# buwantaiji/DominantSparseEigenAD

Hardware: AMD Instinct MI355X
Metric: DominantSparseSymeig fwd+bwd ms & HBM GB/s (TFIM, fp64) (higher is better)
Workload: dtype f64

## Files before the change

dominantsparseeigenad_amd/csrc/dsea_kernels.hip:

```cpp
#include <hip/hip_runtime.h>
#include <hip/hip_ext.h>
#include <stdint.h>

#include <type_traits>

#include "dsea_internal.h"
#include "dsea_device.h"

namespace dsea {

__global__ __launch_bounds__(256) void k_finalize1(const double* __restrict__ partials, int count,
                                                   double* __restrict__ out) {
  __shared__ double sm4[4];
  double acc = 0.0;
  for (int b = threadIdx.x; b < count; b += 256) acc += partials[b];
  double t = block_sum(acc, sm4);
  if (threadIdx.x == 0) out[0] = t;
}

__global__ __launch_bounds__(256) void k_finalize_pair(const double* __restrict__ PA, int na, double* __restrict__ outA,
                                                       const double* __restrict__ PB, int nb, double* __restrict__ outB,
                                                       const double* __restrict__ skipB) {
  __shared__ double sm4[4];
  const bool second = blockIdx.x == 1;
  if (second && skipB && skipB[0] != 0.0) return;
  const double* __restrict__ P = second ? PB : PA;
  const int count = second ? nb : na;
  double acc = 0.0;
  for (int b = threadIdx.x; b < count; b += 256) acc += P[b];
  double t = block_sum(acc, sm4);
  if (threadIdx.x == 0) (second ? outB : outA)[0] = t;
}

template <bool GATE>
__global__ __launch_bounds__(256) void k_finalize_multi(const double* __restrict__ P, int64_t pstride,
                                                        int nw, double* __restrict__ c,
                                                        const double* __restrict__ brk,
                                                        const double* __restrict__ gate) {
  __shared__ double sm4[4];
  const double gate0 = GATE ? gate[0] : 1.0;
  if (broken(brk)) return;
  if (GATE && gate0 == 0.0) return;
  const int j = blockIdx.x;
  const double* __restrict__ row = P + (int64_t)j * pstride;
  double a0 = 0.0, a1 = 0.0, a2 = 0.0, a3 = 0.0;
  int w = threadIdx.x;
  for (; w + 768 < nw; w += 1024) {
    a0 += row[w];
    a1 += row[w + 256];
    a2 += row[w + 512];
    a3 += row[w + 768];
  }
  for (; w < nw; w += 256) a0 += row[w];
  double t = block_sum((a0 + a1) + (a2 + a3), sm4);
  if (threadIdx.x == 0) c[j] = t;
}

template <int NP>
struct RdotsPre {
  double2 uu[NP], qa[NP], qb[NP];
};

template <int RPL, bool GUARD, bool PRE, bool USCALE = false>
__device__ __forceinline__ void rdots_tile(const double* __restrict__ Q, int64_t ldq, int i, int ii, int64_t n,
                                           int64_t base, int lane, const double* __restrict__ u,
                                           double a, double b, double* __restrict__ r,
                                           double* __restrict__ sP, bool accumulate, bool want_rr,
                                           const RdotsPre<RPL / 2>& pre, double usc = 1.0) {
  constexpr int NP = RPL / 2;
  double2 rv[NP];
  const double* __restrict__ q1 = Q + (int64_t)(i - 1) * ldq;
  const double* __restrict__ q2 = (i >= 2) ? Q + (int64_t)(i - 2) * ldq : nullptr;
#pragma unroll
  for (int t = 0; t < NP; ++t) {
    const int64_t row = base + t * 128 + lane * 2;
    double2 uu, qa, qb;
    if (PRE) {
      uu = pre.uu[t];
      qa = pre.qa[t];
      qb = pre.qb[t];
    } else {
      uu = ld2<GUARD>(u, row, n);
      qa = ld2<GUARD>(q1, row, n);
      qb = make_double2(0.0, 0.0);
      if (q2) qb = ld2<GUARD>(q2, row, n);
    }
    if (USCALE) {
      uu.x = uu.x / usc;
      uu.y = uu.y / usc;
    }
    rv[t].x = __dsub_rn(__dsub_rn(uu.x, __dmul_rn(a, qa.x)), __dmul_rn(b, qb.x));
    rv[t].y = __dsub_rn(__dsub_rn(uu.y, __dmul_rn(a, qa.y)), __dmul_rn(b, qb.y));
  }
  if (want_rr) {
    double acc = 0.0;
#pragma unroll
    for (int t = 0; t < NP; ++t) {
      acc = fma(rv[t].x, rv[t].x, acc);
      acc = fma(rv[t].y, rv[t].y, acc);
    }
    acc = wave_sum(acc);
    if (lane == 0) sP[i] = accumulate ? (sP[i] + acc) : acc;
  }
  const int nchunks = ii / 4;
  const bool rev = (i & 1) != 0;
  auto single = [&](int j) {
    const double* __restrict__ qj = Q + (int64_t)j * ldq;
    double acc = 0.0;
#pragma unroll
    for (int t = 0; t < NP; ++t) {
      double2 q = ld2_stream<GUARD>(qj, base + t * 128 + lane * 2, n);
      acc = fma(q.x, rv[t].x, acc);
      acc = fma(q.y, rv[t].y, acc);
    }
    acc = wave_sum(acc);
    if (lane == 0) sP[j] = accumulate ? (sP[j] + acc) : acc;
  };
  if (rev)
    for (int j = ii - 1; j >= 4 * nchunks; --j) single(j);
  for (int cc = 0; cc < nchunks; ++cc) {
    const int j = 4 * (rev ? nchunks - 1 - cc : cc);
    const double* __restrict__ qj = Q + (int64_t)j * ldq;
    double2 q[4][NP];
#pragma unroll
    for (int v = 0; v < 4; ++v)
#pragma unroll
      for (int t = 0; t < NP; ++t) q[v][t] = ld2_stream<GUARD>(qj + (int64_t)v * ldq, base + t * 128 + lane * 2, n);
    double acc[4];
#pragma unroll
    for (int v = 0; v < 4; ++v) {
      acc[v] = 0.0;
#pragma unroll
      for (int t = 0; t < NP; ++t) {
        acc[v] = fma(q[v][t].x, rv[t].x, acc[v]);
        acc[v] = fma(q[v][t].y, rv[t].y, acc[v]);
      }
    }
    const double bsum = wave_sum4_rows(acc[0], acc[1], acc[2], acc[3]);
    if ((lane & 15) == 15) {
      const int idx = j + (lane >> 4);
      sP[idx] = accumulate ? (sP[idx] + bsum) : bsum;
    }
  }
  if (!rev)
    for (int j = 4 * nchunks; j < ii; ++j) single(j);
#pragma unroll
  for (int t = 0; t < NP; ++t) st2<GUARD>(r, base + t * 128 + lane * 2, n, rv[t]);
}

template <int RPL, bool SEL = false, bool USCALE = false>
__global__ __launch_bounds__(256) void k_rdots(const double* __restrict__ Q, int64_t ldq, int i,
                                               int64_t n, const double* __restrict__ u,
                                               const double* __restrict__ alpha,
                                               const double* __restrict__ beta, double* __restrict__ r,
                                               double* __restrict__ P, int64_t pstride, int nw,
                                               int64_t ntiles, const double* __restrict__ aP, int aCount,
                                               double* __restrict__ a_store, int want_rr,
                                               double* __restrict__ brk, const double* __restrict__ sel,
                                               int sel_exit, const double* __restrict__ uscale) {
  const int lane = threadIdx.x & 63;
  const int wpb = blockDim.x >> 6;
  if (SEL && sel_exit && sel[0] == 0.0) return;
  const int64_t widx = (int64_t)blockIdx.x * wpb + (threadIdx.x >> 6);
  constexpr int64_t TILE = 64 * RPL;
  extern __shared__ double rdots_lds[];
  double* __restrict__ sP = rdots_lds + (threadIdx.x >> 6) * (i + 1);
  const int cnt = i + (want_rr ? 1 : 0);
  RdotsPre<RPL / 2> pre;
  const bool pre_ok = widx < nw && widx * TILE + TILE <= n;
  if (pre_ok) {
    const double* __restrict__ q1 = Q + (int64_t)(i - 1) * ldq;
    const double* __restrict__ q2 = (i >= 2) ? Q + (int64_t)(i - 2) * ldq : nullptr;
#pragma unroll
    for (int t = 0; t < RPL / 2; ++t) {
      const int64_t row = widx * TILE + t * 128 + lane * 2;
      pre.uu[t] = ld2<false>(u, row, n);
      pre.qa[t] = ld2<false>(q1, row, n);
      pre.qb[t] = make_double2(0.0, 0.0);
      if (q2) pre.qb[t] = ld2<false>(q2, row, n);
    }
  }
  if (broken(brk)) return;
  if (widx < nw) {
    double a;
    if (aCount > 0) {
      a = sum_partials_wave(aP, aCount, lane);
      if (widx == 0 && lane == 0) a_store[0] = a;
    } else {
      a = alpha[0];
    }
    const double b = beta ? beta[0] : 0.0;
    const double usc = USCALE ? uscale[0] : 1.0;
    if (brk && widx == 0 && lane == 0) brk[1] = fmax(brk[1], fmax(fabs(a), fabs(b)));
    const int ii = (SEL && sel[0] == 0.0) ? 0 : i;
    bool first = true;
    for (int64_t tile = widx; tile < ntiles; tile += nw) {
      const int64_t base = tile * TILE;
      if (first && pre_ok)
        rdots_tile<RPL, false, true, USCALE>(Q, ldq, i, ii, n, base, lane, u, a, b, r, sP, false, want_rr != 0, pre, usc);
      else if (base + TILE <= n)
        rdots_tile<RPL, false, false, USCALE>(Q, ldq, i, ii, n, base, lane, u, a, b, r, sP, !first, want_rr != 0, pre, usc);
      else
        rdots_tile<RPL, true, false, USCALE>(Q, ldq, i, ii, n, base, lane, u, a, b, r, sP, !first, want_rr != 0, pre, usc);
      first = false;
    }
  } else {
    for (int idx = lane; idx < cnt; idx += 64) sP[idx] = 0.0;
  }
  __syncthreads();
  const int row0 = (SEL && sel[0] == 0.0) ? i : 0;
  for (int idx = row0 + threadIdx.x; idx < cnt; idx += blockDim.x) {
    double t = rdots_lds[idx];
    for (int w = 1; w < wpb; ++w) t += rdots_lds[w * (i + 1) + idx];
    P[(int64_t)idx * pstride + blockIdx.x] = t;
  }
}

template <int RPL, bool GUARD, int MODE>
__device__ __forceinline__ double axpy_tile(const double* __restrict__ Q, int64_t ldq, int i, int64_t n,
                                            int64_t base, int lane, const double* __restrict__ c,
                                            double* __restrict__ r) {
  constexpr int NP = RPL / 2;
  double2 w[NP];
#pragma unroll
  for (int t = 0; t < NP; ++t) w[t] = make_double2(0.0, 0.0);
#pragma unroll 4
  for (int jj = 0; jj < i; ++jj) {
    const int j = i - 1 - jj;
    const double* __restrict__ qj = Q + (int64_t)j * ldq;
    const double cj = c[j];
#pragma unroll
    for (int t = 0; t < NP; ++t) {
      const int64_t row = base + t * 128 + lane * 2;
      double2 q = ld2_stream<GUARD>(qj, row, n);
      w[t].x = fma(cj, q.x, w[t].x);
      w[t].y = fma(cj, q.y, w[t].y);
    }
  }
  double acc = 0.0;
#pragma unroll
  for (int t = 0; t < NP; ++t) {
    const int64_t row = base + t * 128 + lane * 2;
    if (MODE == 0) {
      double2 rv = ld2<GUARD>(r, row, n);
      rv.x -= w[t].x;
      rv.y -= w[t].y;
      st2<GUARD>(r, row, n, rv);
      acc = fma(rv.x, rv.x, acc);
      acc = fma(rv.y, rv.y, acc);
    } else {
      st2<GUARD>(r, row, n, w[t]);
    }
  }
  return acc;
}

template <int RPL, int MODE, bool SEL = false>
__global__ __launch_bounds__(256) void k_axpy_norm(const double* __restrict__ Q, int64_t ldq, int i,
                                                   int64_t n, const double* __restrict__ c,
                                                   double* __restrict__ r, double* __restrict__ P,
                                                   int nw, int64_t ntiles, const double* __restrict__ brk,
                                                   const double* __restrict__ sel) {
  const int lane = threadIdx.x & 63;
  const int64_t widx = (int64_t)blockIdx.x * 4 + (threadIdx.x >> 6);
  if (widx >= nw) return;
  const double sel0 = SEL ? sel[0] : 1.0;
  if (broken(brk)) return;
  if (SEL && sel0 == 0.0) {
    if (MODE == 0 && lane == 0) P[widx] = (widx == 0) ? c[i] : 0.0;
    return;
  }
  constexpr int64_t TILE = 64 * RPL;
  double acc = 0.0;
  for (int64_t tile = widx; tile < ntiles; tile += nw) {
    const int64_t base = tile * TILE;
    if (base + TILE <= n)
      acc += axpy_tile<RPL, false, MODE>(Q, ldq, i, n, base, lane, c, r);
    else
      acc += axpy_tile<RPL, true, MODE>(Q, ldq, i, n, base, lane, c, r);
  }
  if (MODE == 0) {
    acc = wave_sum(acc);
    if (lane == 0) P[widx] = acc;
  }
}

template <int W, int NT, bool SEL = false>
__global__ __launch_bounds__(W * 64) void k_rdots_split(const double* __restrict__ Q, int64_t ldq, int i,
                                                        int64_t n, const double* __restrict__ u,
                                                        const double* __restrict__ alpha,
                                                        const double* __restrict__ beta, double* __restrict__ r,
                                                        double* __restrict__ P, int64_t pstride,
                                                        const double* __restrict__ aP, int aCount,
                                                        double* __restrict__ a_store, int want_rr,
                                                        double* __restrict__ brk, const double* __restrict__ sel,
                                                        int sel_exit) {
  if (SEL && sel_exit && sel[0] == 0.0) return;
  const int lane = threadIdx.x & 63, wv = threadIdx.x >> 6;
// ... 776 lines not shown
    if (row != row0) v = ld2<true>(r, row, n);
    v.x = v.x / beta;
    v.y = v.y / beta;
    st2<true>(fa.q_out, row, n, v);
    if (fa.qs_out) st_bf16x2(fa.qs_out, row, n, v);
  }
}

__device__ __forceinline__ double tfim_diag(const TfimParams& p, int64_t i, uint64_t maskL) {
  const uint64_t gi = (uint64_t)(p.row_offset + i);
  const uint64_t rot = ((gi << 1) | (gi >> (p.L - 1))) & maskL;
  const int pop = __popcll(gi ^ rot);
  return p.diag_scale * (double)(-(p.L - 2 * pop));
}

template <int T, bool FUSED>
__global__ __launch_bounds__(256) void k_spmv_tfim(TfimParams p, const double* __restrict__ x,
                                                   double* __restrict__ y,
                                                   const double* __restrict__ shift,
                                                   const double* __restrict__ skip,
                                                   double* __restrict__ P, TfimFusedArgs fa) {
  constexpr int TILE = 1 << T;
  constexpr int NPAIR = TILE / 2;
  constexpr int PER = (NPAIR + 255) / 256;
#ifndef DSEA_FB_FUSED
#define DSEA_FB_FUSED 7
#endif
#ifndef DSEA_FB_PLAIN
#define DSEA_FB_PLAIN 9
#endif
  constexpr int FB = PER >= 4 ? (FUSED ? DSEA_FB_FUSED : DSEA_FB_PLAIN) : (PER == 2 ? 12 : 14);
  __shared__ double2 tile2[NPAIR];
  __shared__ double sm5[5];
  if (!FUSED && skip && skip[0] != 0.0) return;
  if (FUSED && broken(fa.brk)) return;
  const uint64_t maskL = (p.L >= 64) ? ~0ull : ((1ull << p.L) - 1ull);
  const int64_t ntiles = ((int64_t)1 << p.L_local) >> T;
  double acc = 0.0;
  double beta = 1.0, g = 0.0, s = 0.0;
  bool first = true;
  for (int64_t tile = blockIdx.x; tile < ntiles; tile += gridDim.x) {
    const int64_t base = tile * TILE;
    double2 own[PER];
    double2 fb[PER][FB];
#pragma unroll
    for (int t = 0; t < PER; ++t) {
      const int lp = t * 256 + threadIdx.x;
      const int64_t i0 = base + 2 * (int64_t)(lp < NPAIR ? lp : 0);
      own[t] = *reinterpret_cast<const double2*>(x + i0);
#pragma unroll
      for (int e = 0; e < FB; ++e) {
        fb[t][e] = make_double2(0.0, 0.0);
        if (T + e < p.L_local) fb[t][e] = *reinterpret_cast<const double2*>(x + (i0 ^ ((int64_t)1 << (T + e))));
      }
    }
    if (first) {
      if (FUSED && !fused_beta(fa, sm5, beta)) return;
      g = p.g_dev ? p.g_dev[0] : p.g_const;
      s = shift ? shift[0] : 0.0;
      first = false;
    }
    __syncthreads();
#pragma unroll
    for (int t = 0; t < PER; ++t) {
      const int lp = t * 256 + threadIdx.x;
      if (lp < NPAIR) {
        double2 v = own[t];
        if (FUSED) {
          v.x = v.x / beta;
          v.y = v.y / beta;
          *reinterpret_cast<double2*>(fa.q_out + base + 2 * lp) = v;
          if (fa.qs_out)
            *reinterpret_cast<uint32_t*>(fa.qs_out + base + 2 * lp) =
                (uint32_t)f64_to_bf16(v.x) | ((uint32_t)f64_to_bf16(v.y) << 16);
        }
        tile2[lp] = v;
      }
    }
    __syncthreads();
    double2 far[PER];
#pragma unroll
    for (int t = 0; t < PER; ++t) {
      far[t] = make_double2(0.0, 0.0);
#pragma unroll
      for (int e = 0; e < FB; ++e) {
        far[t].x += fb[t][e].x;
        far[t].y += fb[t][e].y;
      }
    }
    int j = T + FB;
    for (; j + 4 <= p.L_local; j += 4) {
      double2 nb[PER][4];
#pragma unroll
      for (int t = 0; t < PER; ++t) {
        const int lp = t * 256 + threadIdx.x;
        const int64_t i0 = base + 2 * (int64_t)(lp < NPAIR ? lp : 0);
#pragma unroll
        for (int e = 0; e < 4; ++e)
          nb[t][e] = *reinterpret_cast<const double2*>(x + (i0 ^ ((int64_t)1 << (j + e))));
      }
#pragma unroll
      for (int t = 0; t < PER; ++t) {
        far[t].x += (nb[t][0].x + nb[t][1].x) + (nb[t][2].x + nb[t][3].x);
        far[t].y += (nb[t][0].y + nb[t][1].y) + (nb[t][2].y + nb[t][3].y);
      }
    }
    for (; j < p.L_local; ++j) {
#pragma unroll
      for (int t = 0; t < PER; ++t) {
        const int lp = t * 256 + threadIdx.x;
        const int64_t i0 = base + 2 * (int64_t)(lp < NPAIR ? lp : 0);
        const double2 nbv = *reinterpret_cast<const double2*>(x + (i0 ^ ((int64_t)1 << j)));
        far[t].x += nbv.x;
        far[t].y += nbv.y;
      }
    }
#pragma unroll
    for (int t = 0; t < PER; ++t) {
      const int lp = t * 256 + threadIdx.x;
      if (lp < NPAIR) {
        const int64_t i0 = base + 2 * (int64_t)lp;
        const double2 xv = tile2[lp];
        double2 sum = make_double2(xv.y, xv.x);
#pragma unroll
        for (int jb = 1; jb < T; ++jb) {
          const double2 nbv = tile2[lp ^ (1 << (jb - 1))];
          sum.x += nbv.x;
          sum.y += nbv.y;
        }
        if (FUSED) {
          sum.x += far[t].x / beta;
          sum.y += far[t].y / beta;
        } else {
          sum.x += far[t].x;
          sum.y += far[t].y;
        }
        double2 v;
        v.x = __dsub_rn(__dmul_rn(xv.x, tfim_diag(p, i0, maskL)), __dmul_rn(g, sum.x));
        v.y = __dsub_rn(__dmul_rn(xv.y, tfim_diag(p, i0 + 1, maskL)), __dmul_rn(g, sum.y));
        if (!FUSED && shift) {
          v.x = __dsub_rn(v.x, __dmul_rn(s, xv.x));
          v.y = __dsub_rn(v.y, __dmul_rn(s, xv.y));
        }
        *reinterpret_cast<double2*>(y + i0) = v;
        acc = fma(xv.x, v.x, acc);
        acc = fma(xv.y, v.y, acc);
      }
    }
  }
  if (P) {
    __syncthreads();
    double tot = block_sum(acc, sm5);
    if (threadIdx.x == 0) P[blockIdx.x] = tot;
  }
}

__global__ void k_spmv_tfim_single(TfimParams p, const double* __restrict__ x, double* __restrict__ y,
                                   const double* __restrict__ shift, const double* __restrict__ skip,
                                   double* __restrict__ P) {
  if (skip && skip[0] != 0.0) return;
  const uint64_t maskL = (p.L >= 64) ? ~0ull : ((1ull << p.L) - 1ull);
  const double xi = x[0];
  double v = __dmul_rn(xi, tfim_diag(p, 0, maskL));
  if (shift) v = __dsub_rn(v, __dmul_rn(shift[0], xi));
  y[0] = v;
  if (P) P[0] = xi * v;
}

__global__ __launch_bounds__(256) void k_cg_update_fused(double* __restrict__ x, double* __restrict__ r,
                                                         const double* __restrict__ d,
                                                         const double* __restrict__ Ad,
                                                         const double* __restrict__ state, int parity,
                                                         const double* __restrict__ dP, int dCount,
                                                         int64_t n, double* __restrict__ P) {
  __shared__ double sm5[5];
  const int64_t stride = (int64_t)gridDim.x * 512;
  const int64_t row0 = ((int64_t)blockIdx.x * 256 + threadIdx.x) * 2;
  double2 xv = ld2<true>(x, row0, n), rv = ld2<true>(r, row0, n);
  double2 dv = ld2<true>(d, row0, n), av = ld2<true>(Ad, row0, n);
  if (state[DSEA_CG_DONE] != 0.0) return;
  const double dAd = sum_partials_block(dP, dCount, sm5);
  const double alpha = state[parity ? DSEA_CG_RRNEW : DSEA_CG_RR] / dAd;
  double acc = 0.0;
  for (int64_t row = row0; row < n; row += stride) {
    if (row != row0) {
      xv = ld2<true>(x, row, n);
      rv = ld2<true>(r, row, n);
      dv = ld2<true>(d, row, n);
      av = ld2<true>(Ad, row, n);
    }
    xv.x = __dadd_rn(xv.x, __dmul_rn(alpha, dv.x));
    xv.y = __dadd_rn(xv.y, __dmul_rn(alpha, dv.y));
    rv.x = __dsub_rn(rv.x, __dmul_rn(alpha, av.x));
    rv.y = __dsub_rn(rv.y, __dmul_rn(alpha, av.y));
    st2<true>(x, row, n, xv);
    st2<true>(r, row, n, rv);
    acc = fma(rv.x, rv.x, acc);
    acc = fma(rv.y, rv.y, acc);
  }
  __syncthreads();
  double t = block_sum(acc, sm5);
  if (threadIdx.x == 0) P[blockIdx.x] = t;
}

__global__ __launch_bounds__(256) void k_cg_direction_fused(const double* __restrict__ r,
                                                            double* __restrict__ d,
                                                            double* __restrict__ state, int parity,
                                                            const double* __restrict__ rP, int rCount,
                                                            double eps, int64_t n) {
  __shared__ double sm5[5];
  const int64_t stride = (int64_t)gridDim.x * 512;
  const int64_t row0 = ((int64_t)blockIdx.x * 256 + threadIdx.x) * 2;
  double2 rv = ld2<true>(r, row0, n), dv = ld2<true>(d, row0, n);
  if (state[DSEA_CG_DONE] != 0.0) return;
  const double rr_new = sum_partials_block(rP, rCount, sm5);
  const double rr = state[parity ? DSEA_CG_RRNEW : DSEA_CG_RR];
  const double rn = sqrt(rr_new);
  const bool conv = rn < eps;
  if (blockIdx.x == 0 && threadIdx.x == 0) {
    state[DSEA_CG_ITERS] += 1.0;
    state[DSEA_CG_RESNORM] = rn;
    if (conv) state[DSEA_CG_DONE] = 1.0;
    else state[parity ? DSEA_CG_RR : DSEA_CG_RRNEW] = rr_new;
  }
  if (conv) return;
  const double beta = rr_new / rr;
  for (int64_t row = row0; row < n; row += stride) {
    if (row != row0) {
      rv = ld2<true>(r, row, n);
      dv = ld2<true>(d, row, n);
    }
    dv.x = __dadd_rn(rv.x, __dmul_rn(beta, dv.x));
    dv.y = __dadd_rn(rv.y, __dmul_rn(beta, dv.y));
    st2<true>(d, row, n, dv);
  }
}

template <int G>
__global__ __launch_bounds__(256) void k_spmv_csr(CsrParams p, const double* __restrict__ x,
                                                  double* __restrict__ y,
                                                  const double* __restrict__ shift,
                                                  const double* __restrict__ skip,
                                                  double* __restrict__ P) {
  __shared__ double sm4[4];
  if (skip && skip[0] != 0.0) return;
  const double s = shift ? shift[0] : 0.0;
  const int sub = threadIdx.x % G;
  const int64_t rows_per_block = 256 / G;
  double acc = 0.0;
  for (int64_t row = (int64_t)blockIdx.x * rows_per_block + threadIdx.x / G; row < p.n;
       row += (int64_t)gridDim.x * rows_per_block) {
    const int64_t lo = p.rowptr[row], hi = p.rowptr[row + 1];
    double sum = 0.0;
    for (int64_t e = lo + sub; e < hi; e += G) sum = fma(p.vals[e], x[p.colidx[e]], sum);
#pragma unroll
    for (int m = G / 2; m >= 1; m >>= 1) sum += __shfl_xor(sum, m, 64);
    if (sub == 0) {
      const double xi = x[row];
      double v = sum;
      if (shift) v = __dsub_rn(v, __dmul_rn(s, xi));
      y[row] = v;
      acc = fma(xi, v, acc);
    }
  }
  if (P) {
    double tot = block_sum(acc, sm4);
    if (threadIdx.x == 0) P[blockIdx.x] = tot;
  }
}

#define CSR_ROWS 128
#define CSR_CAP 6144
__global__ __launch_bounds__(256) void k_spmv_csr_stream(CsrParams p, const double* __restrict__ x,
                                                         double* __restrict__ y,
                                                         const double* __restrict__ shift,
                                                         const double* __restrict__ skip,
                                                         double* __restrict__ P) {
  __shared__ double prod[CSR_CAP];
  __shared__ double sm4[4];
  if (skip && skip[0] != 0.0) return;
  const double s = shift ? shift[0] : 0.0;
  double acc = 0.0;
  const int64_t nchunks = (p.n + CSR_ROWS - 1) / CSR_ROWS;
  for (int64_t chunk = blockIdx.x; chunk < nchunks; chunk += gridDim.x) {
    const int64_t r0 = chunk * CSR_ROWS;
    const int64_t r1 = (r0 + CSR_ROWS < p.n) ? r0 + CSR_ROWS : p.n;
    const int64_t e0 = p.rowptr[r0], e1 = p.rowptr[r1];
    __syncthreads();
    if (e1 - e0 <= CSR_CAP) {
      for (int64_t e = e0 + threadIdx.x; e < e1; e += 256) prod[e - e0] = p.vals[e] * x[p.colidx[e]];
      __syncthreads();
      const int64_t row = r0 + threadIdx.x;
      if (threadIdx.x < CSR_ROWS && row < r1) {
        const int lo = (int)(p.rowptr[row] - e0), hi = (int)(p.rowptr[row + 1] - e0);
        double sum = 0.0;
        for (int e = lo; e < hi; ++e) sum += prod[e];
        const double xi = x[row];
        double v = sum;
        if (shift) v = __dsub_rn(v, __dmul_rn(s, xi));
        y[row] = v;
        acc = fma(xi, v, acc);
      }
    } else {
      const int sub = threadIdx.x & 31;
      for (int64_t row = r0 + (threadIdx.x >> 5); row < r1; row += 8) {
        double sum = 0.0;
// ... 1354 lines not shown
  const double* nullc = nullptr;
  if (g.split_w) {
    const unsigned tiles = (unsigned)g.ntiles;
    EventPair* ev = nullptr;
    switch (g.split_w) {
      case 4: KLAUNCH(ev, (k_axpy_norm_split<4, 1>), tiles, 256, st, Q, ldq, k, n, s, out, nullP, nullc, nullc); break;
      case 8: KLAUNCH(ev, (k_axpy_norm_split<8, 1>), tiles, 512, st, Q, ldq, k, n, s, out, nullP, nullc, nullc); break;
      default: KLAUNCH(ev, (k_axpy_norm_split<16, 1>), tiles, 1024, st, Q, ldq, k, n, s, out, nullP, nullc, nullc); break;
    }
    return;
  }
  const int grid = (g.nw + 3) / 4;
  switch (g.rpl) {
    case 2: hipLaunchKernelGGL((k_axpy_norm<2, 1>), dim3(grid), dim3(256), 0, st, Q, ldq, k, n, s, out, nullP, g.nw, g.ntiles, nullc, nullc); break;
    case 4: hipLaunchKernelGGL((k_axpy_norm<4, 1>), dim3(grid), dim3(256), 0, st, Q, ldq, k, n, s, out, nullP, g.nw, g.ntiles, nullc, nullc); break;
    case 8: hipLaunchKernelGGL((k_axpy_norm<8, 1>), dim3(grid), dim3(256), 0, st, Q, ldq, k, n, s, out, nullP, g.nw, g.ntiles, nullc, nullc); break;
    default: hipLaunchKernelGGL((k_axpy_norm<16, 1>), dim3(grid), dim3(256), 0, st, Q, ldq, k, n, s, out, nullP, g.nw, g.ntiles, nullc, nullc); break;
  }
}

__global__ __launch_bounds__(256) void k_probe_read(const double* __restrict__ x, int64_t n, double* __restrict__ P) {
  __shared__ double sm4[4];
  double acc = 0.0;
  for (int64_t base = (int64_t)blockIdx.x * 4096; base < n; base += (int64_t)gridDim.x * 4096) {
    double2 v[8];
#pragma unroll
    for (int t = 0; t < 8; ++t) v[t] = ld2_stream<true>(x, base + t * 512 + threadIdx.x * 2, n);
#pragma unroll
    for (int t = 0; t < 8; ++t) acc += v[t].x + v[t].y;
  }
  const double tot = block_sum(acc, sm4);
  if (threadIdx.x == 0) P[blockIdx.x] = tot;
}

__global__ __launch_bounds__(256) void k_probe_copy(const double* __restrict__ x, double* __restrict__ y, int64_t n) {
  for (int64_t base = (int64_t)blockIdx.x * 4096; base < n; base += (int64_t)gridDim.x * 4096) {
    double2 v[8];
#pragma unroll
    for (int t = 0; t < 8; ++t) v[t] = ld2_stream<true>(x, base + t * 512 + threadIdx.x * 2, n);
#pragma unroll
    for (int t = 0; t < 8; ++t) st2<true>(y, base + t * 512 + threadIdx.x * 2, n, v[t]);
  }
}

void launch_probe(const double* x, double* y, int64_t n, double* P, int nP, hipStream_t st) {
  int64_t tiles = (n + 4095) / 4096;
  const int grid = (int)(tiles < nP ? tiles : nP);
  if (y)
    hipLaunchKernelGGL(k_probe_copy, dim3(grid), dim3(256), 0, st, x, y, n);
  else
    hipLaunchKernelGGL(k_probe_read, dim3(grid), dim3(256), 0, st, x, n, P);
}

void launch_dot(const double* x, const double* y, int64_t n, double* P, double* out, hipStream_t st) {
  const int nb = ew_blocks(n);
  hipLaunchKernelGGL(k_dot, dim3(nb), dim3(256), 0, st, x, y, n, P);
  launch_finalize1(P, nb, out, st);
}

void launch_shift_dot(const double* x, double* y, const double* shift, const double* skip, int64_t n,
                      double* P, double* out, hipStream_t st) {
  const int nb = ew_blocks(n);
  hipLaunchKernelGGL(k_shift_dot, dim3(nb), dim3(256), 0, st, x, y, shift, skip, n, P);
  hipLaunchKernelGGL(k_cg_finalize_slot, dim3(1), dim3(256), 0, st, (const double*)P, nb, out, skip);
}

int launch_shift_dot_partials(const double* x, double* y, const double* shift, const double* skip, int64_t n, double* P,
                              hipStream_t st) {
  const int nb = ew_blocks(n);
  hipLaunchKernelGGL(k_shift_dot, dim3(nb), dim3(256), 0, st, x, y, shift, skip, n, P);
  return nb;
}

void launch_axpy(double a_host, const double* a_dev, const double* x, double* y, int64_t n,
                 hipStream_t st) {
  hipLaunchKernelGGL(k_axpy, dim3(ew_blocks(n)), dim3(256), 0, st, a_host, a_dev, x, y, n);
}

void launch_scale_store_fused(const double* r, const double* nP, int nCount, double* q, uint16_t* qs, double* beta_store,
                              int64_t n, hipStream_t st) {
  TfimFusedArgs fa = {nP, nCount, q, qs, beta_store, nullptr, 0};
  hipLaunchKernelGGL(k_scale_store_fused, dim3(ew_blocks(n)), dim3(256), 0, st, r, fa, n);
}

int launch_dot_partials(const double* x, const double* y, int64_t n, double* P, hipStream_t st) {
  const int nb = ew_blocks(n);
  hipLaunchKernelGGL(k_dot, dim3(nb), dim3(256), 0, st, x, y, n, P);
  return nb;
}

void launch_scale_store(const double* r, const double* nrm2, double* q, double* beta_out, int64_t n,
                        hipStream_t st, uint16_t* qs, double* brk, int step) {
  hipLaunchKernelGGL(k_scale_store, dim3(ew_blocks(n)), dim3(256), 0, st, r, nrm2, q, beta_out, n, qs, brk, step);
}

void launch_project_apply(const double* v, const double* a, const double* dot, double* out, int64_t n,
                          hipStream_t st) {
  hipLaunchKernelGGL(k_project_apply, dim3(ew_blocks(n)), dim3(256), 0, st, v, a, dot, out, n);
}

void launch_cg_init(const double* b, const double* Ax0, double* r, double* d, double* state, int64_t n,
                    double* P, hipStream_t st) {
  const int nb = tile_blocks(n);
  hipLaunchKernelGGL(k_cg_state_clear, dim3(1), dim3(64), 0, st, state);
  hipLaunchKernelGGL(k_cg_init, dim3(nb), dim3(256), 0, st, b, Ax0, r, d, n, P);
  launch_finalize1(P, nb, state + DSEA_CG_RR, st);
}

void launch_cg_init_check(double* state, double eps, hipStream_t st) {
  hipLaunchKernelGGL(k_cg_init_check, dim3(1), dim3(1), 0, st, state, eps);
}

void launch_cg_update(double* x, double* r, const double* d, const double* Ad, double* state, int64_t n,
                      double* P, hipStream_t st) {
  const int nb = ew_blocks(n);
  hipLaunchKernelGGL(k_cg_update, dim3(nb), dim3(256), 0, st, x, r, d, Ad, (const double*)state, n, P);
  hipLaunchKernelGGL(k_cg_finalize_rrnew, dim3(1), dim3(256), 0, st, (const double*)P, nb, state);
}

int launch_pcg_update(double* x, double* r, double* p, double* s, const double* w, const double* state, int64_t n,
                      double* P, hipStream_t st) {
  const int nb = ew_blocks(n);
  hipLaunchKernelGGL(k_pcg_update, dim3(nb), dim3(256), 0, st, x, r, p, s, w, state, n, P);
  return nb;
}

void launch_pcg_scalars(double* state, const double* pair, double eps, int first, hipStream_t st) {
  hipLaunchKernelGGL(k_pcg_scalars, dim3(1), dim3(1), 0, st, state, pair, eps, first);
}

void launch_cg_check(double* state, double eps, hipStream_t st) {
  hipLaunchKernelGGL(k_cg_check, dim3(1), dim3(1), 0, st, state, eps);
}

void launch_cg_direction(const double* r, double* d, const double* state, int64_t n, hipStream_t st) {
  hipLaunchKernelGGL(k_cg_direction, dim3(ew_blocks(n)), dim3(256), 0, st, r, d, state, n);
}

int launch_spmv(const OpDesc& op, const double* x, double* y, const double* shift, const double* skip,
                double* P, hipStream_t st, EventPair* ev) {
  switch (op.kind) {
    case OP_TFIM: {
      const TfimParams& p = op.tfim;
      if (p.L_local == 0) {
        KLAUNCH(ev, k_spmv_tfim_single, 1, 1, st, p, x, y, shift, skip, P);
        return 1;
      }
      const int T = p.L_local < op.tune_tile_log2 ? p.L_local : op.tune_tile_log2;
      int64_t nb = ((int64_t)1 << p.L_local) >> T;
      if (nb > DSEA_MAX_TFIM_BLOCKS) nb = DSEA_MAX_TFIM_BLOCKS;
      TfimFusedArgs fa = {nullptr, 0, nullptr, nullptr, nullptr, nullptr, 0};
#define TFIM_CASE(TT) \
  case TT: KLAUNCH(ev, (k_spmv_tfim<TT, false>), (unsigned)nb, 256, st, p, x, y, shift, skip, P, fa); break;
      switch (T) {
        TFIM_CASE(1) TFIM_CASE(2) TFIM_CASE(3) TFIM_CASE(4) TFIM_CASE(5) TFIM_CASE(6)
        TFIM_CASE(7) TFIM_CASE(8) TFIM_CASE(9) TFIM_CASE(10) TFIM_CASE(11) TFIM_CASE(12)
        default: return -1;
      }
#undef TFIM_CASE
      return (int)nb;
    }
    case OP_CSR: {
      const CsrParams& p = op.csr;
      const double avg = p.n > 0 ? (double)p.nnz / (double)p.n : 1.0;
      if (op.tune_csr_group == 0 && avg >= 4.0 && avg * CSR_ROWS <= CSR_CAP) {
        int64_t nbs = (p.n + CSR_ROWS - 1) / CSR_ROWS;
        if (nbs > DSEA_MAX_TFIM_BLOCKS) nbs = DSEA_MAX_TFIM_BLOCKS;
        KLAUNCH(ev, k_spmv_csr_stream, (unsigned)nbs, 256, st, p, x, y, shift, skip, P);
        return (int)nbs;
      }
      int G = 4;
      while (G < 64 && G < avg) G *= 2;
      if (op.tune_csr_group) G = op.tune_csr_group;
      const int64_t rows_per_block = 256 / G;
      int64_t nb = (p.n + rows_per_block - 1) / rows_per_block;
      if (nb > DSEA_MAX_EW_BLOCKS) nb = DSEA_MAX_EW_BLOCKS;
      if (nb < 1) nb = 1;
      switch (G) {
        case 4: KLAUNCH(ev, (k_spmv_csr<4>), (unsigned)nb, 256, st, p, x, y, shift, skip, P); break;
        case 8: KLAUNCH(ev, (k_spmv_csr<8>), (unsigned)nb, 256, st, p, x, y, shift, skip, P); break;
        case 16: KLAUNCH(ev, (k_spmv_csr<16>), (unsigned)nb, 256, st, p, x, y, shift, skip, P); break;
        case 32: KLAUNCH(ev, (k_spmv_csr<32>), (unsigned)nb, 256, st, p, x, y, shift, skip, P); break;
        default: KLAUNCH(ev, (k_spmv_csr<64>), (unsigned)nb, 256, st, p, x, y, shift, skip, P); break;
      }
      return (int)nb;
    }
    case OP_SELL: {
      const SellParams& p = op.sell;
      int64_t nb = (p.nslices + 3) / 4;
      if (nb > DSEA_MAX_TFIM_BLOCKS) nb = DSEA_MAX_TFIM_BLOCKS;
      if (nb < 1) nb = 1;
      TfimFusedArgs fa0 = {nullptr, 0, nullptr, nullptr, nullptr, nullptr, 0};
#define SELL_GO(F, M, U, C) KLAUNCH(ev, (k_spmv_sell<F, M, U, C>), (unsigned)nb, 256, st, p, x, y, shift, skip, P, fa0)
      const bool c16 = p.col16 != nullptr;
#define SELL_P2(M) KLAUNCH(ev, (k_spmv_sell<false, M, 8, true, false, false, true>), (unsigned)nb, 256, st, p, x, y, shift, skip, P, fa0)
      if (p.pack2) {
        if (p.mode == 1) SELL_P2(1); else if (p.mode == 2) SELL_P2(2); else SELL_P2(0);
      } else if (p.mode == 1) {
        if (c16) SELL_GO(false, 1, 8, true); else SELL_GO(false, 1, 4, false);
      } else if (p.mode == 2) {
        if (c16) SELL_GO(false, 2, 8, true); else SELL_GO(false, 2, 4, false);
      } else if (c16) {
        if (p.code8) KLAUNCH(ev, (k_spmv_sell<false, 0, 8, true, false, true>), (unsigned)nb, 256, st, p, x, y, shift, skip, P, fa0);
        else if (p.nt) KLAUNCH(ev, (k_spmv_sell<false, 0, 8, true, true>), (unsigned)nb, 256, st, p, x, y, shift, skip, P, fa0);
        else SELL_GO(false, 0, 8, true);
      } else {
        switch (op.tune_sell_unroll) {
          case 1: KLAUNCH(ev, (k_spmv_sell_r5<false>), (unsigned)nb, 256, st, p, x, y, shift, skip, P, fa0); break;
          case 2: SELL_GO(false, 0, 2, false); break;
          case 8: SELL_GO(false, 0, 8, false); break;
          default: SELL_GO(false, 0, 4, false);
        }
      }
#undef SELL_GO
#undef SELL_P2
      return (int)nb;
    }
    case OP_SYMDENSE: {
      const SymDenseParams& p = op.symdense;
      if (p.elem == 4)
        KLAUNCH(ev, k_symv_upper<float>, dim3(p.nb, p.nb), 256, st, p, x, skip);
      else
        KLAUNCH(ev, k_symv_upper<double>, dim3(p.nb, p.nb), 256, st, p, x, skip);
      int64_t nbr = p.nb;
      if (nbr > DSEA_MAX_EW_BLOCKS) nbr = DSEA_MAX_EW_BLOCKS;
      hipLaunchKernelGGL(k_symv_reduce, dim3((unsigned)nbr), dim3(256), 0, st, p, x, y, shift, skip, P);
      return (int)nbr;
    }
    case OP_DENSE:
    case OP_TRANSFER: {
      if (blas_apply(op, x, y, st) != 0) return -1;
      if (!shift && !P) return 0;
      const int nbk = ew_blocks(op.n);
      hipLaunchKernelGGL(k_shift_dot, dim3(nbk), dim3(256), 0, st, x, y, shift, skip, op.n, P);
      return P ? nbk : 0;
    }
    case OP_STENCIL3: {
      const Stencil3Params& p = op.st3;
      const int64_t nb = tile_blocks(p.n);
      TfimFusedArgs fa0 = {nullptr, 0, nullptr, nullptr, nullptr, nullptr, 0};
      KLAUNCH(ev, (k_spmv_stencil3<false>), (unsigned)nb, 256, st, p, x, y, shift, skip, P, fa0);
      return (int)nb;
    }
  }
  return -1;
}

int launch_tfim_fused(const OpDesc& op, const double* r, const double* nP, int nCount, double* q_out, double* y,
                      double* beta_store, double* P, hipStream_t st, EventPair* ev, uint16_t* qs_out, double* brk,
                      int step) {
  TfimFusedArgs fa = {nP, nCount, q_out, qs_out, beta_store, brk, step};
  const double* nullc = nullptr;
  if (op.kind == OP_SELL) {
    const SellParams& p = op.sell;
    int64_t nb = (p.nslices + 3) / 4;
    if (nb > DSEA_MAX_TFIM_BLOCKS) nb = DSEA_MAX_TFIM_BLOCKS;
    if (p.mode != 0) return -1;
#define SELL_GO(U, C) KLAUNCH(ev, (k_spmv_sell<true, 0, U, C>), (unsigned)nb, 256, st, p, r, y, nullc, nullc, P, fa)
    if (p.pack2) {
      KLAUNCH(ev, (k_spmv_sell<true, 0, 8, true, false, false, true>), (unsigned)nb, 256, st, p, r, y, nullc, nullc, P, fa);
    } else if (p.col16) {
      if (p.code8) KLAUNCH(ev, (k_spmv_sell<true, 0, 8, true, false, true>), (unsigned)nb, 256, st, p, r, y, nullc, nullc, P, fa);
      else if (p.nt) KLAUNCH(ev, (k_spmv_sell<true, 0, 8, true, true>), (unsigned)nb, 256, st, p, r, y, nullc, nullc, P, fa);
      else SELL_GO(8, true);
    } else {
      switch (op.tune_sell_unroll) {
        case 1: KLAUNCH(ev, (k_spmv_sell_r5<true>), (unsigned)nb, 256, st, p, r, y, nullc, nullc, P, fa); break;
        case 2: SELL_GO(2, false); break;
        case 8: SELL_GO(8, false); break;
        default: SELL_GO(4, false);
      }
    }
#undef SELL_GO
    return (int)nb;
  }
  if (op.kind == OP_STENCIL3) {
    const Stencil3Params& p = op.st3;
    const int64_t nb = tile_blocks(p.n);
    KLAUNCH(ev, (k_spmv_stencil3<true>), (unsigned)nb, 256, st, p, r, y, nullc, nullc, P, fa);
    return (int)nb;
  }
  if (op.kind != OP_TFIM) return -1;
  const TfimParams& p = op.tfim;
  if (p.L_local == 0) return -1;
  const int T = p.L_local < op.tune_tile_log2 ? p.L_local : op.tune_tile_log2;
  int64_t nb = ((int64_t)1 << p.L_local) >> T;
  if (nb > DSEA_MAX_TFIM_BLOCKS) nb = DSEA_MAX_TFIM_BLOCKS;
#define TFIM_FCASE(TT) \
  case TT: KLAUNCH(ev, (k_spmv_tfim<TT, true>), (unsigned)nb, 256, st, p, r, y, nullc, nullc, P, fa); break;
  switch (T) {
    TFIM_FCASE(1) TFIM_FCASE(2) TFIM_FCASE(3) TFIM_FCASE(4) TFIM_FCASE(5) TFIM_FCASE(6)
    TFIM_FCASE(7) TFIM_FCASE(8) TFIM_FCASE(9) TFIM_FCASE(10) TFIM_FCASE(11) TFIM_FCASE(12)
    default: return -1;
  }
#undef TFIM_FCASE
  return (int)nb;
}

int launch_sell_update_vals(const OpDesc& op, const int64_t* rowptr, const double* vals_csr, hipStream_t st) {
  const SellParams& p = op.sell;
  int64_t nb = (p.nslices + 3) / 4;
  if (nb > DSEA_MAX_TFIM_BLOCKS) nb = DSEA_MAX_TFIM_BLOCKS;
  const int cap = sell_seg_cap(p);
  hipLaunchKernelGGL(k_sell_update_vals, dim3((unsigned)nb), dim3(256), (size_t)cap * 4 * sizeof(double), st, p, rowptr, vals_csr,
                     const_cast<double*>(p.vals), cap);
  return 0;
}

int launch_sddmm(const OpDesc& op, const int64_t* rowptr, const double* v1, const double* v2, double alpha, int accumulate,
                 bool sym, double* out, hipStream_t st) {
  if (op.kind == OP_SELL) {
    const SellParams& p = op.sell;
    int64_t nb = (p.nslices + 3) / 4;
    if (nb > DSEA_MAX_TFIM_BLOCKS) nb = DSEA_MAX_TFIM_BLOCKS;
    const int cap = sell_seg_cap(p);
#define SDDMM_CASE(M, S)                                                                                                  \
  hipLaunchKernelGGL((k_sell_sddmm<M, S>), dim3((unsigned)nb), dim3(256), (size_t)cap * 4 * sizeof(double), st, p, rowptr, v1, v2, \
                     alpha, accumulate, out, cap)
    if (p.mode == 0) {
      if (sym) SDDMM_CASE(0, true); else SDDMM_CASE(0, false);
    } else if (sym) {
      return -1;
    } else if (p.mode == 1) {
      SDDMM_CASE(1, false);
    } else {
      SDDMM_CASE(2, false);
    }
#undef SDDMM_CASE
    return 0;
  }
  if (op.kind == OP_CSR) {
    const CsrParams& p = op.csr;
    int64_t nb = (p.n + 31) / 32;
    if (nb > DSEA_MAX_EW_BLOCKS) nb = DSEA_MAX_EW_BLOCKS;
    if (nb < 1) nb = 1;
    if (sym) hipLaunchKernelGGL(k_csr_sddmm<true>, dim3((unsigned)nb), dim3(256), 0, st, p, v1, v2, alpha, accumulate, out);
    else hipLaunchKernelGGL(k_csr_sddmm<false>, dim3((unsigned)nb), dim3(256), 0, st, p, v1, v2, alpha, accumulate, out);
    return 0;
  }
  return -1;
}

int launch_cg_update_fused(double* x, double* r, const double* d, const double* Ad, const double* state,
                           int parity, const double* dP, int dCount, int64_t n, double* P, hipStream_t st) {
  const int nb = tile_blocks(n);
  hipLaunchKernelGGL(k_cg_update_fused, dim3(nb), dim3(256), 0, st, x, r, d, Ad, state, parity, dP, dCount, n, P);
  return nb;
}

void launch_cg_direction_fused(const double* r, double* d, double* state, int parity, const double* rP,
                               int rCount, double eps, int64_t n, hipStream_t st) {
  hipLaunchKernelGGL(k_cg_direction_fused, dim3(tile_blocks(n)), dim3(256), 0, st, r, d, state, parity, rP, rCount,
                     eps, n);
}

void launch_axpy_multi_dot(double a_host, const double* a_dev, const double* const* xs, int count,
                           const double* shift, const double* skip, const double* x, double* y, int64_t n,
                           double* P, double* dot_out, hipStream_t st, const double* pendP, int pendN, double* pendOut) {
  MultiSrc ms;
  ms.count = count;
  for (int b = 0; b < 6; ++b) ms.p[b] = b < count ? xs[b] : nullptr;
  const int nb = ew_blocks(n);
  hipLaunchKernelGGL(k_axpy_multi_dot, dim3(nb), dim3(256), 0, st, a_host, a_dev, ms, shift, skip, x, y, n, P);
  if (pendP)
    hipLaunchKernelGGL(k_finalize_pair, dim3(2), dim3(256), 0, st, pendP, pendN, pendOut, (const double*)P, nb, dot_out, skip);
  else
    hipLaunchKernelGGL(k_cg_finalize_slot, dim3(1), dim3(256), 0, st, (const double*)P, nb, dot_out, skip);
}

void launch_form_r(const double* u, const double* q1, const double* q2, const double* alpha, const double* beta,
                   double* r, double* r_copy, int64_t n, hipStream_t st) {
  hipLaunchKernelGGL(k_form_r, dim3(ew_blocks(n)), dim3(256), 0, st, u, q1, q2, alpha, beta, r, r_copy, n);
}

void launch_hypercube_flipsum(const double* xT, double* zT, int P, int p, int64_t chunk, hipStream_t st) {
  int64_t nb = ((int64_t)P * chunk + 255) / 256;
  if (nb > DSEA_MAX_EW_BLOCKS) nb = DSEA_MAX_EW_BLOCKS;
  if (nb < 1) nb = 1;
  hipLaunchKernelGGL(k_hypercube_flipsum, dim3((unsigned)nb), dim3(256), 0, st, xT, zT, P, p, chunk);
}

void launch_plz_finish(const double* r, const double* y, const double* pair, double* q, uint16_t* qs, double* u,
                       double* alpha_out, double* beta_out, int64_t n, hipStream_t st) {
  hipLaunchKernelGGL(k_plz_finish, dim3(ew_blocks(n)), dim3(256), 0, st, r, y, pair, q, qs, u, alpha_out,
                     beta_out, n);
}

void launch_plz_finish_form(double* r, const double* y, const double* pair, double* q, uint16_t* qs, const double* qprev,
                            double* alpha_out, double* beta_out, double* r_copy, int64_t n, hipStream_t st) {
  hipLaunchKernelGGL(k_plz_finish_form, dim3(ew_blocks(n)), dim3(256), 0, st, r, y, pair, q, qs, qprev, alpha_out, beta_out,
                     r_copy, n);
}

void launch_finalize_pair(const double* PA, int na, double* outA, const double* PB, int nb, double* outB,
                          const double* skipB, hipStream_t st) {
  hipLaunchKernelGGL(k_finalize_pair, dim3(2), dim3(256), 0, st, PA, na, outA, PB, nb, outB, skipB);
}

int launch_three_term(const double* u, const double* q1, const double* q2, const double* aP, int aCount,
                      double* a_store, const double* beta, double* r, double* P, double* psi, const double* s1,
                      int64_t n, double* brk, hipStream_t st) {
  const int nb = ew_blocks(n);
  hipLaunchKernelGGL(k_three_term, dim3(nb), dim3(256), 0, st, u, q1, q2, aP, aCount, a_store, beta, r, P, psi, s1, n,
                     brk);
  return nb;
}

void launch_finalize_slot(const double* P, int count, double* out, const double* skip, hipStream_t st) {
  hipLaunchKernelGGL(k_cg_finalize_slot, dim3(1), dim3(256), 0, st, P, count, out, skip);
}

size_t persist_comm_bytes(int64_t n) {
  const int64_t nt = (n + 511) / 512;
  return (size_t)(4 * nt + 20 * 256) * sizeof(unsigned long long);
}
int launch_cg_persist(const OpDesc& op, const double* shift, const double* b, double* x, double* state, double eps,
                      int64_t maxiter, void* comm, int ppt_override, hipStream_t st, int lose_peer) {
  const bool merged = ppt_override >= 100;
  if (merged) ppt_override -= 100;
  if (op.kind != OP_STENCIL3 || op.st3.halo_lo || op.st3.halo_hi) return -1;
  const int64_t n = op.st3.n;
  const int64_t nt = (n + 511) / 512;
  if (nt > DSEA_PERSIST_CG_MAX_TILES) return -1;
  int ppt, nvb = 4;
  switch (ppt_override) {
    case 1: case 2: ppt = ppt_override; break;
    case 21: case 22: ppt = ppt_override - 20; nvb = 2; break;
    case 11: case 12: ppt = ppt_override - 10; nvb = 1; break;
    default:
      if (nt <= 64) { ppt = 1; nvb = 1; }
      else if (nt <= 512) { ppt = 1; nvb = 2; }
      else { ppt = 2; nvb = 2; }
      if (merged && nt > 64 && nt <= 512) { ppt = 2; nvb = 1; }
      break;
  }
  const int tpw = nvb * ppt;
  const int G = (int)((nt + tpw - 1) / tpw);
  if (G > 256) {
    return -1;
  }
  {
    static thread_local int cu_dev = -1, cu_count = 0;
    int dev = 0;
    if (hipGetDevice(&dev) != hipSuccess) return -2;
    if (dev != cu_dev) {
      if (hipDeviceGetAttribute(&cu_count, hipDeviceAttributeMultiprocessorCount, dev) != hipSuccess) return -2;
      cu_dev = dev;
// ... 32 lines not shown
```

Measured before the change: 6086.

## Add 512-thread TFIM SpMV kernel and fold neighbour dots into residual pass

```diff
diff --git a/dominantsparseeigenad_amd/csrc/dsea_kernels.hip b/dominantsparseeigenad_amd/csrc/dsea_kernels.hip
--- a/dominantsparseeigenad_amd/csrc/dsea_kernels.hip
+++ b/dominantsparseeigenad_amd/csrc/dsea_kernels.hip
@@ -71,6 +71,13 @@
   double2 rv[NP];
   const double* __restrict__ q1 = Q + (int64_t)(i - 1) * ldq;
   const double* __restrict__ q2 = (i >= 2) ? Q + (int64_t)(i - 2) * ldq : nullptr;
+#ifdef DSEA_RDOTS_REREAD
+  constexpr bool REG_DOTS = false;
+#else
+  constexpr bool REG_DOTS = true;
+#endif
+  const int nreg = (REG_DOTS && ii == i) ? (i >= 2 ? 2 : 1) : 0;
+  double da = 0.0, db = 0.0;
 #pragma unroll
   for (int t = 0; t < NP; ++t) {
     const int64_t row = base + t * 128 + lane * 2;
@@ -91,6 +98,19 @@
     }
     rv[t].x = __dsub_rn(__dsub_rn(uu.x, __dmul_rn(a, qa.x)), __dmul_rn(b, qb.x));
     rv[t].y = __dsub_rn(__dsub_rn(uu.y, __dmul_rn(a, qa.y)), __dmul_rn(b, qb.y));
+    if (REG_DOTS) {
+      da = fma(qa.x, rv[t].x, da);
+      da = fma(qa.y, rv[t].y, da);
+      db = fma(qb.x, rv[t].x, db);
+      db = fma(qb.y, rv[t].y, db);
+    }
+  }
+  if (nreg > 0) {
+    const double bsum = wave_sum4_rows(da, db, 0.0, 0.0);
+    if (lane == 15 || (nreg == 2 && lane == 31)) {
+      const int idx = i - 1 - (lane >> 4);
+      sP[idx] = accumulate ? (sP[idx] + bsum) : bsum;
+    }
   }
   if (want_rr) {
     double acc = 0.0;
@@ -102,7 +122,8 @@
     acc = wave_sum(acc);
     if (lane == 0) sP[i] = accumulate ? (sP[i] + acc) : acc;
   }
-  const int nchunks = ii / 4;
+  const int ns = ii - nreg;
+  const int nchunks = ns / 4;
   const bool rev = (i & 1) != 0;
   auto single = [&](int j) {
     const double* __restrict__ qj = Q + (int64_t)j * ldq;
@@ -117,7 +138,7 @@
     if (lane == 0) sP[j] = accumulate ? (sP[j] + acc) : acc;
   };
   if (rev)
-    for (int j = ii - 1; j >= 4 * nchunks; --j) single(j);
+    for (int j = ns - 1; j >= 4 * nchunks; --j) single(j);
   for (int cc = 0; cc < nchunks; ++cc) {
     const int j = 4 * (rev ? nchunks - 1 - cc : cc);
     const double* __restrict__ qj = Q + (int64_t)j * ldq;
@@ -143,7 +164,7 @@
     }
   }
   if (!rev)
-    for (int j = 4 * nchunks; j < ii; ++j) single(j);
+    for (int j = 4 * nchunks; j < ns; ++j) single(j);
 #pragma unroll
   for (int t = 0; t < NP; ++t) st2<GUARD>(r, base + t * 128 + lane * 2, n, rv[t]);
 }
@@ -1226,6 +1247,198 @@
     __syncthreads();
     double tot = block_sum(acc, sm5);
     if (threadIdx.x == 0) P[blockIdx.x] = tot;
+  }
+}
+
+__host__ __device__ constexpr int tfim_w_fb_sum(int T, bool fused) {
+  return T >= 11 ? (fused ? DSEA_FB_FUSED : DSEA_FB_PLAIN) : 12;
+}
+__host__ __device__ constexpr int tfim_w_fb_load(int T, bool fused) {
+  return (T >= 11 ? 9 : 12) > tfim_w_fb_sum(T, fused) ? (T >= 11 ? 9 : 12) : tfim_w_fb_sum(T, fused);
+}
+
+template <int T, bool FUSED>
+__global__ __launch_bounds__(512) __attribute__((amdgpu_waves_per_eu(4))) void k_spmv_tfim_w(TfimParams p, const double* __restrict__ x,
+                                                     double* __restrict__ y,
+                                                     const double* __restrict__ shift,
+                                                     const double* __restrict__ skip,
+                                                     double* __restrict__ P, TfimFusedArgs fa) {
+  static_assert(T >= 10, "512 threads own at least one pair each");
+  constexpr int TILE = 1 << T;
+  constexpr int NPAIR = TILE / 2;
+  constexpr int PER = NPAIR / 512;
+  constexpr int FB_SUM = tfim_w_fb_sum(T, FUSED);
+  constexpr int FB_LOAD = tfim_w_fb_load(T, FUSED);
+  __shared__ double2 tile2[NPAIR];
+  __shared__ double2 xchg[256][2 * PER];
+  __shared__ double sm5[5];
+  const int tid = threadIdx.x, h = tid >> 8, l = tid & 255;
+  const int lane = tid & 63, w = tid >> 6;
+  const uint64_t maskL = (p.L >= 64) ? ~0ull : ((1ull << p.L) - 1ull);
+  const int64_t ntiles = ((int64_t)1 << p.L_local) >> T;
+  const int nfar = p.L_local - T;
+  const double stop0 = FUSED ? (fa.brk ? fa.brk[0] : 0.0) : (skip ? skip[0] : 0.0);
+  double acc = 0.0;
+  double beta = 1.0, g = 0.0, s = 0.0;
+  bool first = true;
+  for (int64_t tile = blockIdx.x; tile < ntiles; tile += gridDim.x) {
+    const int64_t base = tile * TILE;
+    double2 own[PER];
+    double2 fb[PER][FB_LOAD];
+#pragma unroll
+    for (int t = 0; t < PER; ++t) {
+      const int lp = (h * PER + t) * 256 + l;
+      const int64_t i0 = base + 2 * (int64_t)lp;
+      own[t] = *reinterpret_cast<const double2*>(x + i0);
+#pragma unroll
+      for (int e = 0; e < FB_LOAD; ++e) {
+        fb[t][e] = make_double2(0.0, 0.0);
+        if (e < nfar) fb[t][e] = *reinterpret_cast<const double2*>(x + (i0 ^ ((int64_t)1 << (T + e))));
+      }
+    }
+    double2 far[PER];
+#pragma unroll
+    for (int t = 0; t < PER; ++t) {
+      far[t] = make_double2(0.0, 0.0);
+#pragma unroll
+      for (int e = 0; e < FB_SUM; ++e) {
+        far[t].x += fb[t][e].x;
+        far[t].y += fb[t][e].y;
+      }
+    }
+#pragma unroll
+    for (int e = FB_SUM; e < FB_LOAD; ++e)
+      if (e < nfar) {
+#pragma unroll
+        for (int t = 0; t < PER; ++t) {
+          far[t].x += fb[t][e].x;
+          far[t].y += fb[t][e].y;
+        }
+      }
+    int j = T + FB_LOAD;
+    if (first) {
+      if (stop0 != 0.0) return;
+      if (FUSED) {
+        double a0 = 0.0, a1 = 0.0;
+        if (h == 0) {
+          int b = l;
+          for (; b + 256 < fa.nCount; b += 512) {
+            a0 += fa.nP[b];
+            a1 += fa.nP[b + 256];
+          }
+          if (b < fa.nCount) a0 += fa.nP[b];
+        }
+        const double v = wave_sum(a0 + a1);
+        if (lane == 0 && w < 4) sm5[w] = v;
+        __syncthreads();
+        if (tid == 0) sm5[4] = ((sm5[0] + sm5[1]) + sm5[2]) + sm5[3];
+        __syncthreads();
+        beta = sqrt(sm5[4]);
+        if (blockIdx.x == 0 && tid == 0) fa.beta_store[0] = beta;
+        if (fa.brk && !(beta > DSEA_BREAK_TOL * fa.brk[1])) {
+          if (blockIdx.x == 0 && tid == 0) fa.brk[0] = (double)fa.step;
+          return;
+        }
+      }
+      g = p.g_dev ? p.g_dev[0] : p.g_const;
+      s = shift ? shift[0] : 0.0;
+      first = false;
+    }
+    __syncthreads();
+#pragma unroll
+    for (int t = 0; t < PER; ++t) {
+      const int lp = (h * PER + t) * 256 + l;
+      double2 v = own[t];
+      if (FUSED) {
+        v.x = v.x / beta;
+        v.y = v.y / beta;
+        *reinterpret_cast<double2*>(fa.q_out + base + 2 * lp) = v;
+        if (fa.qs_out)
+          *reinterpret_cast<uint32_t*>(fa.qs_out + base + 2 * lp) =
+              (uint32_t)f64_to_bf16(v.x) | ((uint32_t)f64_to_bf16(v.y) << 16);
+      }
+      tile2[lp] = v;
+    }
+    __syncthreads();
+    for (; j + 4 <= p.L_local; j += 4) {
+      double2 nb[PER][4];
+#pragma unroll
+      for (int t = 0; t < PER; ++t) {
+        const int64_t i0 = base + 2 * (int64_t)((h * PER + t) * 256 + l);
+#pragma unroll
+        for (int e = 0; e < 4; ++e)
+          nb[t][e] = *reinterpret_cast<const double2*>(x + (i0 ^ ((int64_t)1 << (j + e))));
+      }
+#pragma unroll
+      for (int t = 0; t < PER; ++t) {
+        far[t].x += (nb[t][0].x + nb[t][1].x) + (nb[t][2].x + nb[t][3].x);
+        far[t].y += (nb[t][0].y + nb[t][1].y) + (nb[t][2].y + nb[t][3].y);
+      }
+    }
+    for (; j < p.L_local; ++j) {
+#pragma unroll
+      for (int t = 0; t < PER; ++t) {
+        const int64_t i0 = base + 2 * (int64_t)((h * PER + t) * 256 + l);
+        const double2 nbv = *reinterpret_cast<const double2*>(x + (i0 ^ ((int64_t)1 << j)));
+        far[t].x += nbv.x;
+        far[t].y += nbv.y;
+      }
+    }
+#pragma unroll
+    for (int t = 0; t < PER; ++t) {
+      const int lp = (h * PER + t) * 256 + l;
+      const int64_t i0 = base + 2 * (int64_t)lp;
+      const double2 xv = tile2[lp];
+      double2 sum = make_double2(xv.y, xv.x);
+#pragma unroll
+      for (int jb = 1; jb < T; ++jb) {
+        const double2 nbv = tile2[lp ^ (1 << (jb - 1))];
+        sum.x += nbv.x;
+        sum.y += nbv.y;
+      }
+      if (FUSED) {
+        sum.x += far[t].x / beta;
+        sum.y += far[t].y / beta;
+      } else {
+        sum.x += far[t].x;
+        sum.y += far[t].y;
+      }
+      double2 v;
+      v.x = __dsub_rn(__dmul_rn(xv.x, tfim_diag(p, i0, maskL)), __dmul_rn(g, sum.x));
+      v.y = __dsub_rn(__dmul_rn(xv.y, tfim_diag(p, i0 + 1, maskL)), __dmul_rn(g, sum.y));
+      if (!FUSED && shift) {
+        v.x = __dsub_rn(v.x, __dmul_rn(s, xv.x));
+        v.y = __dsub_rn(v.y, __dmul_rn(s, xv.y));
+      }
+      *reinterpret_cast<double2*>(y + i0) = v;
+      if (P) {
+        if (h == 0) {
+          acc = fma(xv.x, v.x, acc);
+          acc = fma(xv.y, v.y, acc);
+        } else {
+          xchg[l][2 * t] = xv;
+          xchg[l][2 * t + 1] = v;
+        }
+      }
+    }
+    if (P) {
+      __syncthreads();
+      if (h == 0) {
+#pragma unroll
+        for (int t = 0; t < PER; ++t) {
+          const double2 xv = xchg[l][2 * t], v = xchg[l][2 * t + 1];
+          acc = fma(xv.x, v.x, acc);
+          acc = fma(xv.y, v.y, acc);
+        }
+      }
+    }
+  }
+  if (P) {
+    __syncthreads();
+    const double v = wave_sum(acc);
+    if (lane == 0 && w < 4) sm5[w] = v;
+    __syncthreads();
+    if (tid == 0) P[blockIdx.x] = ((sm5[0] + sm5[1]) + sm5[2]) + sm5[3];
   }
 }
 
@@ -2886,11 +3099,18 @@
       TfimFusedArgs fa = {nullptr, 0, nullptr, nullptr, nullptr, nullptr, 0};
 #define TFIM_CASE(TT) \
   case TT: KLAUNCH(ev, (k_spmv_tfim<TT, false>), (unsigned)nb, 256, st, p, x, y, shift, skip, P, fa); break;
+#ifndef DSEA_TFIM_V1
+#define TFIM_WCASE(TT) \
+  case TT: KLAUNCH(ev, (k_spmv_tfim_w<TT, false>), (unsigned)nb, 512, st, p, x, y, shift, skip, P, fa); break;
+#else
+#define TFIM_WCASE(TT) TFIM_CASE(TT)
+#endif
       switch (T) {
         TFIM_CASE(1) TFIM_CASE(2) TFIM_CASE(3) TFIM_CASE(4) TFIM_CASE(5) TFIM_CASE(6)
-        TFIM_CASE(7) TFIM_CASE(8) TFIM_CASE(9) TFIM_CASE(10) TFIM_CASE(11) TFIM_CASE(12)
+        TFIM_CASE(7) TFIM_CASE(8) TFIM_CASE(9) TFIM_WCASE(10) TFIM_WCASE(11) TFIM_CASE(12)
         default: return -1;
       }
+#undef TFIM_WCASE
 #undef TFIM_CASE
       return (int)nb;
     }
@@ -3022,11 +3242,23 @@
   if (nb > DSEA_MAX_TFIM_BLOCKS) nb = DSEA_MAX_TFIM_BLOCKS;
 #define TFIM_FCASE(TT) \
   case TT: KLAUNCH(ev, (k_spmv_tfim<TT, true>), (unsigned)nb, 256, st, p, r, y, nullc, nullc, P, fa); break;
+#ifndef DSEA_TFIM_V1
+#define TFIM_FWCASE(TT) \
+  case TT: KLAUNCH(ev, (k_spmv_tfim_w<TT, true>), (unsigned)nb, 512, st, p, r, y, nullc, nullc, P, fa); break;
+#else
+#define TFIM_FWCASE(TT) TFIM_FCASE(TT)
+#endif
+  const bool wide = p.L_local - T <= tfim_w_fb_load(T, true) || tfim_w_fb_load(T, true) == tfim_w_fb_sum(T, true);
+  if (!wide && T == 11) {
+    KLAUNCH(ev, (k_spmv_tfim<11, true>), (unsigned)nb, 256, st, p, r, y, nullc, nullc, P, fa);
+    return (int)nb;
+  }
   switch (T) {
     TFIM_FCASE(1) TFIM_FCASE(2) TFIM_FCASE(3) TFIM_FCASE(4) TFIM_FCASE(5) TFIM_FCASE(6)
-    TFIM_FCASE(7) TFIM_FCASE(8) TFIM_FCASE(9) TFIM_FCASE(10) TFIM_FCASE(11) TFIM_FCASE(12)
+    TFIM_FCASE(7) TFIM_FCASE(8) TFIM_FCASE(9) TFIM_FWCASE(10) TFIM_FWCASE(11) TFIM_FCASE(12)
     default: return -1;
   }
+#undef TFIM_FWCASE
 #undef TFIM_FCASE
   return (int)nb;
 }
```

After: 6097, median of 4. Within noise of the previous version (+0.2%).
